# ViTAE-Transformer/SAMRS

Hardware: AMD Instinct MI355X
Metric: images/sec (1024^2, vit_h, 32 boxes/img) SAM box->mask (higher is better)
Workload: dtype f16

## Files before the change

### include/samrs_hip.h

```cpp
#ifndef SAMRS_HIP_H
#define SAMRS_HIP_H

#include <stdint.h>

#ifdef __cplusplus
extern "C" {
#endif

#define SAMRS_ABI_VERSION 5

enum samrs_status {
    SAMRS_OK = 0,
    SAMRS_ERR_NOT_SET = -1,
    SAMRS_ERR_BAD_SHAPE = -2,
    SAMRS_ERR_BAD_ARG = -3,
    SAMRS_ERR_HIP = -4,
    SAMRS_ERR_BAD_WEIGHTS = -5,
    SAMRS_ERR_CAPACITY = -6,
    SAMRS_ERR_PRECISION = -7,
    SAMRS_ERR_RANGE = -8
};

enum samrs_precision {
    SAMRS_PREC_BF16 = 0,
// ... 39 lines not shown
int samrs_predict(samrs_engine_t* e, int slot, int n_prompts,
                  const float* boxes, const float* point_coords, const int32_t* point_labels,
                  int n_points, const float* mask_input, int multimask, int return_logits,
                  int in_h, int in_w, int orig_h, int orig_w,
                  void* masks_out, float* iou_out, float* lowres_out, void* stream);

int samrs_predict_multi(samrs_engine_t* e, int n_images, const int* slots, const int* prompt_offsets,
                        const float* boxes, const float* point_coords, const int32_t* point_labels, int n_points,
                        const float* mask_input, int multimask, int return_logits,
                        const int* in_hw, const int* orig_hw, void* const* masks_out, float* iou_out, float* lowres_out,
                        void* stream);

int samrs_paint(samrs_engine_t* e, const uint8_t* masks, const int32_t* labels, int n,
                int orig_h, int orig_w, uint8_t* seg_mask, int64_t* areas_out,
                int64_t* class_pixels, int64_t* class_instances, int n_classes, void* stream);

int samrs_select_best(samrs_engine_t* e, const uint8_t* masks, const float* iou, int n, int n_sel, int h, int w,
                      uint8_t* best_out, float* quality_out, int64_t* areas_out, void* stream);

int samrs_gt_match(samrs_engine_t* e, const uint8_t* masks, int n, int h, int w, const uint8_t* label_rgb,
                   const uint8_t* colors, int64_t* inter_out, int64_t* gt_area_out, uint8_t* gt_masks_out, void* stream);

int samrs_rle_encode(samrs_engine_t* e, const uint8_t* masks, int n, int h, int w, uint8_t* out, int64_t out_capacity,
                     int64_t* cursor, int64_t* table, void* stream);

int samrs_scene_claim(samrs_engine_t* e, const uint8_t* masks, const int32_t* ranks, const int32_t* labels, int n, int h, int w,
                      int x0, int y0, int H, int W, int32_t* order, int64_t* areas_out,
                      int64_t* class_pixels, int64_t* class_instances, int n_classes, void* stream);
int samrs_scene_resolve(samrs_engine_t* e, const int32_t* order, const int32_t* labels_by_rank, int n_ranks, int H, int W,
                        uint8_t* seg, void* stream);
// ... 48 lines not shown
```

### samrs_amd/csrc/decoder_kernels.hip

```cpp
#include "common.h"
#include "kernels.h"
#include "postprocess_value.h"

namespace {

constexpr float TWO_PI = 6.283185307179586f;

__device__ __forceinline__ float pe_channel(const float* __restrict__ gauss, float cx01, float cy01, int ch, int half) {
    const int f = ch < half ? ch : ch - half;
    const float vx = 2.0f * cx01 - 1.0f, vy = 2.0f * cy01 - 1.0f;
    const float a = TWO_PI * (vx * gauss[f] + vy * gauss[half + f]);
    return ch < half ? sinf(a) : cosf(a);
}

__global__ void prompt_tokens_kernel(PromptParams p, float* __restrict__ tokens, float* __restrict__ tokens2, int T, int C) {
    const int j = blockIdx.x, b = blockIdx.y, ch = threadIdx.x;
    const int half = C / 2;
    const bool has_pts = p.point_coords != nullptr;
    const bool has_box = p.boxes != nullptr;
    const int npt = has_pts ? p.n_points + (has_box ? 0 : 1) : 0;
    float v;
    if (j == 0) {
        v = p.iou_token[ch];
    } else if (j < 5) {
// ... 168 lines not shown
#pragma unroll
            for (int c = 0; c < DH; ++c) acc[c] = acc[c] * corr + pj * vr[c];
            m = mn;
        }
        const float inv = 1.0f / l;
        float* orow = o + ((size_t)b * T + i) * C + h * DH;
#pragma unroll
        for (int c = 0; c < DH; ++c) orow[c] = acc[c] * inv;
    }
}

constexpr int T2I_TG = 8;
constexpr int T2I_REC = 10;
constexpr float T2I_NEG = -1.0e30f;

template <int PREC>
__global__ __launch_bounds__(256, 2) void t2i_partial_kernel(const float* __restrict__ qp, const uint16_t* __restrict__ kp,
                                                          const uint16_t* __restrict__ vp, int ld, long bstride,
                                                          const int* __restrict__ slot_of, float* __restrict__ part, int T, int tokens, int Ci, int kpw) {
    __shared__ float sm[4][T2I_TG][16][T2I_REC];
    const int split = blockIdx.x, b = blockIdx.y, t0 = blockIdx.z * T2I_TG;
    const int lane = threadIdx.x & 63, wave = threadIdx.x >> 6;
    const int ch = lane & 15, kq = lane >> 4;
    float q[T2I_TG][8], acc[T2I_TG][8], m[T2I_TG], l[T2I_TG];
#pragma unroll
    for (int t = 0; t < T2I_TG; ++t) {
        m[t] = T2I_NEG;
        l[t] = 0.f;
        const bool tv = t0 + t < T;
        const float* qr = qp + ((size_t)b * T + (tv ? t0 + t : 0)) * Ci + ch * 8;
#pragma unroll
        for (int c = 0; c < 8; ++c) {
            q[t][c] = tv ? qr[c] * (0.25f * 1.44269504088896340736f) : 0.f;
            acc[t][c] = 0.f;
        }
    }
    const int kbeg = (split * 4 + wave) * kpw;
    const int kend = kbeg + kpw < tokens ? kbeg + kpw : tokens;
    const int kbat = slot_of ? slot_of[b] : b;
    const uint16_t* kb = kp + (size_t)kbat * bstride * ld + ch * 8;
    const uint16_t* vb = vp + (size_t)kbat * bstride * ld + ch * 8;
// ... 13 lines not shown
        T2I_LOAD(kn, vn, k0 + 4 * U)
#pragma unroll
        for (int u = 0; u < U; ++u) {
            const bool valid = k0 + 4 * u + kq < kend;
            const uint32_t kw[4] = {kk[u].x, kk[u].y, kk[u].z, kk[u].w};
            const uint32_t vw[4] = {vv[u].x, vv[u].y, vv[u].z, vv[u].w};
            float kf[8], vf[8];
#pragma unroll
            for (int c = 0; c < 4; ++c) {
                kf[2 * c] = ET<PREC>::to_float((uint16_t)(kw[c] & 0xffffu));
                kf[2 * c + 1] = ET<PREC>::to_float((uint16_t)(kw[c] >> 16));
                vf[2 * c] = ET<PREC>::to_float((uint16_t)(vw[c] & 0xffffu));
                vf[2 * c + 1] = ET<PREC>::to_float((uint16_t)(vw[c] >> 16));
            }
#pragma unroll
            for (int t = 0; t < T2I_TG; ++t) {
                float sc = 0.f;
#pragma unroll
                for (int c = 0; c < 8; ++c) sc += q[t][c] * kf[c];
                sc += __builtin_bit_cast(float, __builtin_amdgcn_update_dpp(0, __builtin_bit_cast(int, sc), 0xB1, 0xF, 0xF, true));
                sc = valid ? sc : T2I_NEG;
                const float mn = fmaxf(m[t], sc);
                const float corr = __builtin_amdgcn_exp2f(m[t] - mn);
                const float pj = valid ? __builtin_amdgcn_exp2f(sc - mn) : 0.f;
                l[t] = l[t] * corr + pj;
#pragma unroll
                for (int c = 0; c < 8; ++c) acc[t][c] = acc[t][c] * corr + pj * vf[c];
                m[t] = mn;
            }
        }
#pragma unroll
        for (int u = 0; u < U; ++u) { kk[u] = kn[u]; vv[u] = vn[u]; }
    }
#undef T2I_LOAD
#pragma unroll
    for (int off = 16; off <= 32; off <<= 1) {
#pragma unroll
        for (int t = 0; t < T2I_TG; ++t) {
            const float mo = __shfl_xor(m[t], off, 64), lo = __shfl_xor(l[t], off, 64);
            const float mn = fmaxf(m[t], mo);
            const float fs = __builtin_amdgcn_exp2f(m[t] - mn), fo = __builtin_amdgcn_exp2f(mo - mn);
            l[t] = l[t] * fs + lo * fo;
#pragma unroll
            for (int c = 0; c < 8; ++c) acc[t][c] = acc[t][c] * fs + __shfl_xor(acc[t][c], off, 64) * fo;
            m[t] = mn;
        }
    }
    if (lane < 16) {
#pragma unroll
        for (int t = 0; t < T2I_TG; ++t) {
            float* r = sm[wave][t][ch];
            r[0] = m[t]; r[1] = l[t];
#pragma unroll
            for (int c = 0; c < 8; ++c) r[2 + c] = acc[t][c];
        }
    }
    __syncthreads();
    if (threadIdx.x < T2I_TG * 16) {
        const int t = threadIdx.x >> 4, c16 = threadIdx.x & 15;
        float mm = sm[0][t][c16][0];
#pragma unroll
        for (int w = 1; w < 4; ++w) mm = fmaxf(mm, sm[w][t][c16][0]);
        float ll = 0.f, a[8] = {0.f, 0.f, 0.f, 0.f, 0.f, 0.f, 0.f, 0.f};
#pragma unroll
        for (int w = 0; w < 4; ++w) {
            const float f = __builtin_amdgcn_exp2f(sm[w][t][c16][0] - mm);
            ll += sm[w][t][c16][1] * f;
#pragma unroll
            for (int c = 0; c < 8; ++c) a[c] += sm[w][t][c16][2 + c] * f;
        }
        float* r = part + ((((size_t)b * gridDim.z + blockIdx.z) * gridDim.x + split) * (T2I_TG * 16) + threadIdx.x) * T2I_REC;
        r[0] = mm; r[1] = ll;
#pragma unroll
        for (int c = 0; c < 8; ++c) r[2 + c] = a[c];
    }
}

__global__ __launch_bounds__(T2I_TG * 16) void t2i_merge_kernel(const float* __restrict__ part, float* __restrict__ o,
                                                                int splits, int T, int Ci) {
    const int b = blockIdx.x, tg = blockIdx.y;
    const int t = tg * T2I_TG + (threadIdx.x >> 4), ch = threadIdx.x & 15;
    if (t >= T) return;
    const float* base = part + (((size_t)b * gridDim.y + tg) * splits * (T2I_TG * 16) + threadIdx.x) * T2I_REC;
    const size_t sstride = (size_t)(T2I_TG * 16) * T2I_REC;
    float mm = T2I_NEG;
    for (int s = 0; s < splits; ++s) mm = fmaxf(mm, base[s * sstride]);
// ... 629 lines not shown
    }
}

__global__ void class_stats_kernel(const unsigned long long* __restrict__ areas, const int32_t* __restrict__ labels, int n,
                                   unsigned long long* __restrict__ cpix, unsigned long long* __restrict__ cins, int n_classes) {
    if (threadIdx.x != 0 || blockIdx.x != 0) return;
    for (int j = 0; j < n; ++j) {
        const int l = labels[j];
        if (areas[j] > 0 && l >= 0 && l < n_classes) {
            if (cpix) cpix[l] += areas[j];
            if (cins) cins[l] += 1ull;
        }
    }
}

__global__ void resample_pass_kernel(const uint8_t* __restrict__ in, uint8_t* __restrict__ out, const int32_t* __restrict__ bounds,
                                     const int32_t* __restrict__ coef, int ksize, int in_len, int out_len, int other,
                                     int horizontal) {
    const long t = (long)blockIdx.x * blockDim.x + threadIdx.x;
    const long total = (long)out_len * other * 3;
    if (t >= total) return;
    const int c = t % 3;
    long u = t / 3;
    int o, q;
    if (horizontal) { o = u % out_len; q = u / out_len; } else { q = u % other; o = u / other; }
    const int k0 = bounds[2 * o], kn = bounds[2 * o + 1];
    const int32_t* k = coef + (size_t)o * ksize;
    int ss = 1 << 21;
    for (int i = 0; i < kn; ++i) {
        const size_t idx = horizontal ? ((size_t)q * in_len + (k0 + i)) * 3 + c : ((size_t)(k0 + i) * other + q) * 3 + c;
// ... 163 lines not shown
    if (C / heads != 32 || T > TOK_MAX) return hipErrorInvalidValue;
    token_self_attn_kernel<32><<<n, 256, 3 * T * C * sizeof(float), s>>>(q, k, v, o, T, C, heads);
    return hipGetLastError();
}
size_t t2i_workspace_floats(int n, int T) {
    return (size_t)n * ((T + T2I_TG - 1) / T2I_TG) * T2I_MAX_SPLITS * (T2I_TG * 16) * T2I_REC;
}
hipError_t launch_t2i_attention(int prec, const float* qp, const void* kp, const void* vp, int ld, long bstride,
                                float* o, float* workspace, int n, int T, int tokens, int Ci, int heads, hipStream_t s,
                                const int* slot_of) {
    if (Ci != 128 || heads != 8 || T > TOK_MAX || !workspace) return hipErrorInvalidValue;
    int splits = (tokens + 255) / 256;
    splits = splits < 1 ? 1 : (splits > T2I_MAX_SPLITS ? T2I_MAX_SPLITS : splits);
    const int kpw = ((tokens + splits * 4 - 1) / (splits * 4) + 15) / 16 * 16;
    const int tgs = (T + T2I_TG - 1) / T2I_TG;
    dim3 g(splits, n, tgs), b(256);
    const uint16_t* k = (const uint16_t*)kp;
    const uint16_t* v = (const uint16_t*)vp;
    if (prec == PREC_BF16) t2i_partial_kernel<PREC_BF16><<<g, b, 0, s>>>(qp, k, v, ld, bstride, slot_of, workspace, T, tokens, Ci, kpw);
    else t2i_partial_kernel<PREC_F16><<<g, b, 0, s>>>(qp, k, v, ld, bstride, slot_of, workspace, T, tokens, Ci, kpw);
    t2i_merge_kernel<<<dim3(n, tgs), T2I_TG * 16, 0, s>>>(workspace, o, splits, T, Ci);
    return hipGetLastError();
}
hipError_t launch_i2t_attention(int prec, const void* qi, int ld, long bstride, const float* kt, const float* vt,
                                void* out, int n, int T, int tokens, int Ci, int heads, hipStream_t s) {
    if (Ci / heads != 16 || 256 % heads) return hipErrorInvalidValue;
    const int per = 256 / heads;
    dim3 g((tokens + per - 1) / per, n), b(256);
    const size_t sh = 2 * (size_t)T * heads * I2T_HS * sizeof(float);
    if (prec == PREC_BF16)
        i2t_attention_kernel<PREC_BF16><<<g, b, sh, s>>>((const uint16_t*)qi, ld, bstride, kt, vt, (uint16_t*)out, T, tokens, Ci);
    else
        i2t_attention_kernel<PREC_F16><<<g, b, sh, s>>>((const uint16_t*)qi, ld, bstride, kt, vt, (uint16_t*)out, T, tokens, Ci);
    return hipGetLastError();
}
// ... 64 lines not shown
    const bool fused = seg && areas && hw % 16 == 0 && (((uintptr_t)masks | (uintptr_t)seg) & 15) == 0;
    if (seg && !fused) paint_kernel<<<(int)((hw + 255) / 256), 256, 0, s>>>(masks, labels, n, hw, seg);
    if (areas) {
        HIP_CHECK_RET(hipMemsetAsync(areas, 0, sizeof(unsigned long long) * n, s));
        if (fused) {
            paint_area_kernel<<<(int)((hw / 16 + 255) / 256), 256, 0, s>>>(masks, labels, n, hw, seg, areas);
        } else {
            dim3 g(64, n);
            area_kernel<<<g, 256, 0, s>>>(masks, hw, areas);
        }
        if (class_pixels || class_instances)
            class_stats_kernel<<<1, 64, 0, s>>>(areas, labels, n, class_pixels, class_instances, n_classes);
    }
    return hipGetLastError();
}

hipError_t launch_select_best(const uint8_t* masks, const float* iou, int n, int nsel, int h, int w, uint8_t* out, float* quality,
                              unsigned long long* areas, hipStream_t s) {
    if (n < 1 || nsel < 1 || h < 1 || w < 1) return hipErrorInvalidValue;
    const long hw = (long)h * w;
    HIP_CHECK_RET(hipMemsetAsync(areas, 0, sizeof(unsigned long long) * n, s));
    int chunks = (int)((hw / 16 + 255) / 256);
    chunks = chunks < 1 ? 1 : (chunks > 64 ? 64 : chunks);
    select_best_kernel<<<dim3(chunks, n), 256, 0, s>>>(masks, iou, nsel, hw, out, quality, areas);
    return hipGetLastError();
}

hipError_t launch_gt_match(const uint8_t* masks, int n, int h, int w, const uint8_t* label_rgb, const uint8_t* colors,
                           unsigned long long* inter, unsigned long long* gt_area, uint8_t* gt_masks, hipStream_t s) {
    const long hw = (long)h * w;
// ... 18 lines not shown
```

### samrs_amd/csrc/engine_masks.hip

```cpp
#include <cmath>

#include "engine_state.h"

extern "C" {
int samrs_paint(samrs_engine_t* e, const uint8_t* masks, const int32_t* labels, int n, int h, int w, uint8_t* seg,
                int64_t* areas, int64_t* cpix, int64_t* cins, int n_classes, void* stream) {
    if (!e || !masks || !labels || n < 1 || h < 1 || w < 1) return fail(e, SAMRS_ERR_BAD_ARG, "samrs_paint: bad argument");
    if ((cpix || cins) && !areas) return fail(e, SAMRS_ERR_BAD_ARG, "samrs_paint: class statistics need areas_out");
    ON_DEVICE(e);
    CK(e, launch_paint(masks, labels, n, h, w, seg, (unsigned long long*)areas, (unsigned long long*)cpix,
                       (unsigned long long*)cins, n_classes, (hipStream_t)stream));
    return SAMRS_OK;
}

int samrs_select_best(samrs_engine_t* e, const uint8_t* masks, const float* iou, int n, int n_sel, int h, int w, uint8_t* best_out,
                      float* quality_out, int64_t* areas_out, void* stream) {
    if (!e || !masks || !iou || !best_out || !quality_out || !areas_out || n < 1 || n_sel < 1 || h < 1 || w < 1)
        return fail(e, SAMRS_ERR_BAD_ARG, "samrs_select_best: bad argument");
    ON_DEVICE(e);
    CK(e, launch_select_best(masks, iou, n, n_sel, h, w, best_out, quality_out, (unsigned long long*)areas_out, (hipStream_t)stream));
    return SAMRS_OK;
}
int samrs_gt_match(samrs_engine_t* e, const uint8_t* masks, int n, int h, int w, const uint8_t* label_rgb, const uint8_t* colors,
                   int64_t* inter_out, int64_t* gt_area_out, uint8_t* gt_masks_out, void* stream) {
    if (!e || !masks || !label_rgb || !colors || !inter_out || !gt_area_out || n < 1 || h < 1 || w < 1)
        return fail(e, SAMRS_ERR_BAD_ARG, "samrs_gt_match: bad argument");
// ... 198 lines not shown
```

### samrs_amd/csrc/kernels.h

```cpp
#pragma once
#include <hip/hip_runtime.h>
#include <stdint.h>

struct GemmOpts {
    int ld = 0;
    int gelu_form = 1;
};
hipError_t launch_gemm_et(int prec, const void* A, const void* B, void* C, const float* bias,
                          const float* add2d, int add2d_period, int M, int N, int K, bool out_f32,
                          bool gelu, bool accumulate, hipStream_t s, GemmOpts opts = {});
void gemm_debug_choice(int prec, int M, int N, int K, bool out_f32, bool gelu, bool accumulate, bool has_add2d, int ld, int variant,
                       int32_t* out8);
hipError_t launch_gemm_et_gln(int prec, const void* A, const void* B, void* C, const float* bias, const float* gamma_beta,
                              int M, int N, int K, hipStream_t s, const void* A_lo = nullptr, const void* B_lo = nullptr);
hipError_t launch_gemm_et_stats(int prec, const void* A, const void* B, float* C, const float* bias, void* Xh, float* stats,
                                int M, int N, int K, hipStream_t s);
hipError_t launch_gemm_et_fold(int prec, const void* Xh, const void* Wf, void* C, const float* bias_f, const float* cvec,
                               const float* rowstat, int M, int N, int K, bool gelu, hipStream_t s);
bool gemm_split3_ok(int M, int N, int K, bool out_f32 = false);
hipError_t launch_gemm_et_split3(int prec, const void* A, const void* A_lo, const void* B, const void* B_lo, void* C, const float* bias,
                                 int M, int N, int K, bool out_f32, bool accumulate, hipStream_t s, int split_from_n = 0,
                                 const float* add2d = nullptr, int add2d_period = 0);
void set_gemm_variant(int v);
bool gemm_has_experiments();
// ... 87 lines not shown
                                float* out, float* workspace, int n, int T, int tokens, int Ci, int heads, hipStream_t s,
                                const int* slot_of = nullptr);
hipError_t launch_i2t_attention(int prec, const void* qi, int ld, long batch_stride_rows, const float* kt,
                                const float* vt, void* out, int n, int T, int tokens, int Ci, int heads, hipStream_t s);
hipError_t launch_group_ln_gelu(int prec, const float* in, const float* gamma, const float* beta, float eps,
                                void* out, long rows, int groups, int gsize, hipStream_t s);
hipError_t launch_upscale2_masks(int prec, const void* u1, const void* w, const void* w_lo, const float* bias, const float* hyper,
                                 float* low, int n, int grid, int n_mask_tokens, int sel0, int n_sel, hipStream_t s);
hipError_t launch_mask_product(int prec, const void* up2, const float* hyper, float* low, int n, int grid,
                               int n_mask_tokens, int sel0, int n_sel, hipStream_t s);
hipError_t launch_postprocess(const float* low, int n_masks, int in_h, int in_w, int orig_h, int orig_w,
                              int img_size, int return_logits, void* out, hipStream_t s);
hipError_t launch_paint(const uint8_t* masks, const int32_t* labels, int n, int h, int w, uint8_t* seg,
                        unsigned long long* areas, unsigned long long* class_pixels,
                        unsigned long long* class_instances, int n_classes, hipStream_t s);
hipError_t launch_select_best(const uint8_t* masks, const float* iou, int n, int nsel, int h, int w, uint8_t* out, float* quality,
                              unsigned long long* areas, hipStream_t s);
hipError_t launch_gt_match(const uint8_t* masks, int n, int h, int w, const uint8_t* label_rgb, const uint8_t* colors,
                           unsigned long long* inter, unsigned long long* gt_area, uint8_t* gt_masks, hipStream_t s);
hipError_t launch_resample_pass(const uint8_t* in, uint8_t* out, const int32_t* bounds, const int32_t* coef, int ksize,
                                int in_len, int out_len, int other, int horizontal, hipStream_t s);
hipError_t launch_rbox_prompt(const int32_t* pts, int n, int nv, int h, int w, int th, int tw, int img_size, int out_size,
                              float* out, hipStream_t s,
                              int fill_rule = 0 );
hipError_t launch_i2t_fused(int prec, const void* qi, int ld, long q_bstride, const float* kt, const float* vt, const void* w,
                            const void* w_lo , const float* bias, const float* resid,
                            long r_bstride, const float* gamma, const float* beta, float eps, float* outF, void* outE,
                            void* outE_lo , int n, int T, int tokens, int Ci, int C, hipStream_t s,
                            const int* slot_of = nullptr);

// ... 61 lines not shown
```

### samrs_amd/driver.py

```python
from __future__ import annotations

import contextlib
import os

import queue
import threading
from dataclasses import dataclass, field
from typing import Callable, Iterable, Iterator, List, NamedTuple, Optional, Sequence, Tuple

import numpy as np
import torch


def shard(items: Sequence, rank: int, world: int) -> List:
    return list(sorted(items))[rank::world]


def box_chunks(n: int, batch_size: int) -> List[Tuple[int, int]]:
    out, start = [], 0
    end = min(n, start + batch_size)
    for _ in range(n // batch_size + 1):
        if start < end:
            out.append((start, end))
        start = end
# ... 405 lines not shown
    if need > hi:
        return False, None, f"a chain of {need} prompts exceeds what the engine accepts ({hi})"
    return True, need, f"decode_prompts raised from {capacity} to {need}"


class TilePipeline:

    BOX_WIDTH = 4

    def __init__(self, sam, n_classes: int, batch: int = 8, box_batch: int = 20, keep_masks: bool = False,
                 out_depth: int = 3, max_boxes: int = 512, device_inputs: bool = False, rle: bool = False,
                 rle_buffer_mb: int = 256, precision="auto", _multimask: bool = False, png_lut: Optional[np.ndarray] = None,
                 png_buffer_mb: Optional[int] = None, batch_decode="auto", min_region_area: int = 0,
                 region_mode: str = "both", mask_boxes: bool = False, quality: bool = False, min_stability: float = 0.0,
                 min_pred_iou: float = 0.0, min_inside_box: float = 0.0, polygons: bool = False, polygon_buffer_mb: int = 64,
                 polygon_max_edges: int = 65536):
        from .transforms import ResizeLongestSide
        lut, poly_vertices = validate_output_options(min_region_area, region_mode, polygons, polygon_buffer_mb, polygon_max_edges, png_lut)
        self.min_region_area, self.region_mode = int(min_region_area), region_mode
        self.thresholds = (float(min_stability), float(min_pred_iou), float(min_inside_box))
        if any(t != t or t < 0 for t in self.thresholds):
            raise ValueError("min_stability, min_pred_iou and min_inside_box must be >= 0 (0 = off)")
        self.filter = any(t > 0 for t in self.thresholds)
        self.quality = bool(quality) or self.filter
        eng = sam.engine
        if eng is None:
            raise RuntimeError("move the model to the GPU first: sam.to('cuda')")
        self.split_mode = self._choose_split(sam, precision, multimask=_multimask)
        self.allow_reduced = _multimask and isinstance(precision, int) and not isinstance(precision, bool)
        self.eng = eng
        if self.split_mode is not None:
            with self._mode():
                pass
        if out_depth < 2:
            raise ValueError("out_depth must be >= 2: batch k-1's results are still on loan to the sink when batch k decodes")
        if eng.max_images < 2 * batch:
            raise ValueError(f"TilePipeline(batch={batch}) needs an engine with max_images >= {2 * batch} "
                             f"(two embedding slot sets); got {eng.max_images}")
        self.sam, self.eng, self.dev = sam, eng, eng.device
        self.batch, self.box_batch, self.keep_masks, self.max_boxes = batch, box_batch, keep_masks, max_boxes
        self.rle = rle
        self.batch_decode, self.batch_decode_reason = self._resolve_batch_decode(batch_decode)
        self.batch_decode_on = self.batch_decode
        self.png = png_lut is not None
        self.side = sam.cfg.img_size
        self.transform = ResizeLongestSide(sam.image_encoder.img_size)
        self.class_pixels = torch.zeros(n_classes, dtype=torch.int64, device=self.dev)
        self.class_instances = torch.zeros(n_classes, dtype=torch.int64, device=self.dev)
        dev, side = self.dev, self.side
        self.s_h2d, self.s_enc, self.s_dec = (torch.cuda.Stream(dev) for _ in range(3))
        self.device_inputs = device_inputs
        self.pin_in = None
        if not device_inputs:
            self.pin_in = [torch.empty(batch, side, side, 3, dtype=torch.uint8).pin_memory() for _ in range(2)]
        self.mask_boxes, self.polygons = bool(mask_boxes), bool(polygons)
        self.dev_in = [torch.empty(batch, side, side, 3, dtype=torch.uint8, device=dev) for _ in range(2)]
        bw = self.BOX_WIDTH
        self.pin_box = [torch.empty(batch * max_boxes, bw, dtype=torch.float32).pin_memory() for _ in range(2)]
# ... 154 lines not shown
    def _decode_multi(self, b: int, tiles, offs):
        per = [self._tile_prompts(b, t, hw, off, nb) for (t, hw), (off, nb) in zip(tiles, offs)]
        args = [None if per[0][j] is None else torch.cat([p[j] for p in per]) for j in range(4)]
        masks, iou, low = self.eng.predict_multi([b * self.batch + i for i in range(len(tiles))], [nb for _, nb in offs], *args,
                                               self.multimask, False, [(int(t.shape[0]), int(t.shape[1])) for t, _ in tiles],
                                               [tuple(hw) for _, hw in tiles])
        return list(zip(masks, iou, low))

    def _chunk_masks(self, b: int, i: int, tile, hw, off: int, s: int, e: int, pre):
        if pre is not None:
            return pre[0][s:e], pre[1][s:e], pre[2][s:e]
        in_size = (int(tile.shape[0]), int(tile.shape[1]))
        return self.eng.predict(b * self.batch + i, *self._tile_prompts(b, tile, hw, off + s, e - s), self.multimask, False, in_size,
                                tuple(hw))

    def _decode_tile(self, b: int, i: int, tile, hw, off: int, nb: int, out: _OutBuf, pre=None) -> None:
        eng, (H, W) = self.eng, hw
        in_size = (int(tile.shape[0]), int(tile.shape[1]))
        native = (H, W) == (self.side, self.side)
        seg = self.seg_dev[b][i] if native else torch.full((H, W), 255, dtype=torch.uint8, device=self.dev)
        kept = []
        for s, e in box_chunks(nb, self.box_batch):
            masks, iou, low = self._chunk_masks(b, i, tile, hw, off, s, e, pre)
            if self.quality:
                self._score(b, i, off, s, e, masks[:, 0], iou, low, in_size, (H, W))
            if self.min_region_area:
                eng.clean_masks(masks[:, 0], self.min_region_area, self.region_mode, areas_out=False,
                                changed_out=self.chg_dev[b][i, s:e])
            if self.mask_boxes:
                eng.mask_boxes(masks[:, 0], (0, 0), self.hbox_dev[b][i, s:e], self.rbox_dev[b][i, s:e], self.rec_dev[b][i, s:e])
            if self.polygons:
                eng.mask_polygons(masks[:, 0], (0, 0), self.polygon_max_edges, self.poly_vert_dev[b], self.poly_ring_dev[b],
                                  self.poly_out.cur[b], self.poly_out.tab[b][off + s:off + e])
            eng.paint(masks[:, 0], self.dev_lab[b][off + s:off + e], seg, self.class_pixels, self.class_instances,
                      areas_out=self.area_dev[b][i, s:e])
            if self.rle:
                eng.rle_encode(masks[:, 0], self.rle_dev[b], self.rle_out.cur[b], self.rle_out.tab[b][off + s:off + e])
            if self.keep_masks:
                kept.append(masks[:, 0].view(torch.uint8))
        if self.png and not native:
            eng.png_encode(seg, self.png_lut, self.png_dev[b], self.png_out.cur[b], self.png_out.tab[b][i:i + 1])
        if native:
            out.seg[i].copy_(seg, non_blocking=True)
        else:
            out.odd[i] = seg.cpu()
        out.masks[i] = torch.cat(kept).cpu() if (self.keep_masks and kept) else None

    STABILITY_OFFSET = 1.0

    def _score(self, b: int, i: int, off: int, s: int, e: int, masks, iou, low, in_size, hw) -> None:
        eng = self.eng
        counts = eng.score_masks(low[:, 0], in_size, hw, self.STABILITY_OFFSET, boxes=self.dev_box[b][off + s:off + e],
                                 counts_out=self.cnt_dev[b][i, s:e])
        self.qual_dev[b][i, s:e].copy_(iou[:, 0])
        if self.filter:
            eng.filter_masks(masks, counts, self.qual_dev[b][i, s:e], *self.thresholds, keep_out=self.keep_dev[b][i, s:e])

    def _input_frame_boxes(self, boxes: torch.Tensor, hw, in_size) -> torch.Tensor:
        if tuple(hw) == tuple(in_size):
            return boxes
        return self.transform.apply_boxes_torch(boxes, hw)

    def _decode(self, b: int, items, tiles, offs, out: _OutBuf):
        with torch.cuda.stream(self.s_dec):
            self.s_dec.wait_event(self.ev_enc[b])
            self.seg_dev[b].fill_(255)
            for st in self.streams:
                st.reset(b)
            with self._mode():
                pre = self._decode_multi(b, tiles, offs) if self.batch_decode and sum(nb for _, nb in offs) else None
                for i, ((t, hw), (off, nb)) in enumerate(zip(tiles, offs)):
                    self._decode_tile(b, i, t, hw, off, nb, out, None if pre is None else pre[i])
            if self.png:
                self._encode_png(b, tiles)
            for t in self.tables:
                out.tables[t.field].copy_(getattr(self, t.dev)[b], non_blocking=True)
            for st in self.streams:
                st.copy_table(b, out)
            self.ev_dec[b].record(self.s_dec)
            out.done.record(self.s_dec)

    def _encode_png(self, b: int, tiles) -> None:
        native = [i for i, (_, hw) in enumerate(tiles) if tuple(hw) == (self.side, self.side)]
        runs: List[List[int]] = []
        for i in native:
            if runs and runs[-1][-1] == i - 1:
                runs[-1].append(i)
# ... 199 lines not shown
```

### samrs_amd/engine.py

```python
from __future__ import annotations

import contextlib
import ctypes as C
import os
from typing import Dict, List, Optional, Sequence, Tuple

import numpy as np
import torch

from .synth import SamConfig

_HERE = os.path.dirname(os.path.abspath(__file__))
LIB_PATH = os.path.join(_HERE, "csrc", "libsamrs_hip.so")

PREC_BF16, PREC_F16 = 0, 1
PRECISIONS = {"bf16": PREC_BF16, "f16": PREC_F16, "fp16": PREC_F16}

ABI_VERSION = 5
REGION_MODES = {"holes": 1, "islands": 2, "both": 3}
SPLIT_PATCH, SPLIT_NECK, SPLIT_OI, SPLIT_UP, SPLIT_DEFAULT = 1, 2, 4, 8, 15
SPLIT_ATTN, SPLIT_MLP, SPLIT_ATTN_V, SPLIT_LIN2, SPLIT_ALL = 16, 32, 64, 128, 255

OK, ERR_NOT_SET, ERR_BAD_SHAPE, ERR_BAD_ARG, ERR_HIP, ERR_BAD_WEIGHTS, ERR_CAPACITY, ERR_PRECISION, ERR_RANGE = 0, -1, -2, -3, -4, -5, -6, -7, -8

# ... 31 lines not shown
    lib.samrs_create.argtypes = [C.POINTER(samrs_config), ip, C.c_char_p, ip]
    lib.samrs_destroy.argtypes = [vp]
    lib.samrs_destroy.restype = None
    lib.samrs_last_error.argtypes = [vp]
    lib.samrs_last_error.restype = C.c_char_p
    lib.samrs_load_weight.argtypes = [vp, C.c_char_p, vp, C.POINTER(C.c_int64), ip]
    lib.samrs_finalize_weights.argtypes = [vp, vp]
    lib.samrs_set_images.argtypes = [vp, vp, ip, ip, ip, ip, vp]
    lib.samrs_set_images_ragged.argtypes = [vp, C.POINTER(vp), C.POINTER(ip), C.POINTER(ip), ip, ip, vp]
    lib.samrs_get_embedding.argtypes = [vp, ip, vp, vp]
    lib.samrs_set_embedding.argtypes = [vp, ip, vp, vp]
    lib.samrs_reset_image.argtypes = [vp, ip]
    lib.samrs_predict.argtypes = [vp, ip, ip, vp, vp, vp, ip, vp, ip, ip, ip, ip, ip, ip, vp, vp, vp, vp]
    lib.samrs_predict_multi.argtypes = PREDICT_MULTI_ARGTYPES
    lib.samrs_paint.argtypes = [vp, vp, vp, ip, ip, ip, vp, vp, vp, vp, ip, vp]
    lib.samrs_debug_encoder_prefix.argtypes = [vp, vp, ip, ip, ip, ip, vp, vp]
    lib.samrs_debug_encoder_prefix.restype = ip
    lib.samrs_debug_time_dominant_kernel.argtypes = [vp, ip]
    lib.samrs_debug_time_dominant_kernel.restype = ip
    lib.samrs_debug_dominant_kernel_time.argtypes = [vp, C.POINTER(C.c_float), C.POINTER(ip), C.POINTER(ip), C.POINTER(ip), C.POINTER(ip)]
    lib.samrs_debug_dominant_kernel_time.restype = ip
    lib.samrs_resample_pass_u8.argtypes = [vp, vp, vp, vp, ip, ip, ip, ip, ip, vp]
    lib.samrs_resample_pass_u8.restype = ip
    lib.samrs_rbox_mask_prompt.argtypes = [vp, ip, ip, ip, ip, ip, ip, ip, ip, vp, vp]
    lib.samrs_rbox_mask_prompt.restype = ip
    lib.samrs_rbox_mask_prompt_rule.argtypes = [vp, ip, ip, ip, ip, ip, ip, ip, ip, ip, vp, vp]
    lib.samrs_rbox_mask_prompt_rule.restype = ip
    lib.samrs_k_gemm.argtypes = [ip, vp, vp, vp, vp, vp, ip, ip, ip, ip, ip, ip, ip, vp]
    lib.samrs_k_gemm_f32.argtypes = [vp, ip, vp, vp, vp, ip, ip, ip, ip, ip, ip, vp]
    lib.samrs_k_gemm_stats.argtypes = [ip, vp, vp, vp, vp, vp, vp, ip, ip, ip, vp]
# ... 693 lines not shown
              class_pixels: Optional[torch.Tensor] = None, class_instances: Optional[torch.Tensor] = None,
              areas_out: Optional[torch.Tensor] = None) -> torch.Tensor:
        m = masks.view(torch.uint8) if masks.dtype == torch.bool else masks
        m = m.reshape(-1, m.shape[-2], m.shape[-1]).contiguous()
        n, h, w = m.shape
        labels = labels.to(dtype=torch.int32, device=self.device).contiguous()
        if areas_out is not None:
            assert areas_out.dtype == torch.int64 and areas_out.is_contiguous() and areas_out.numel() == n and areas_out.is_cuda
        areas = areas_out if areas_out is not None else torch.empty(n, dtype=torch.int64, device=self.device)
        ncls = 0 if class_pixels is None else class_pixels.numel()
        with torch.cuda.device(self.device):
            self._check(self.lib.samrs_paint(self.handle, m.data_ptr(), labels.data_ptr(), n, h, w, seg.data_ptr(),
                                             areas.data_ptr(), _ptr(class_pixels), _ptr(class_instances), ncls, _stream()))
        return areas

    def _check_scene(self, rc: int) -> None:
        if rc == ERR_BAD_ARG:
            raise EngineError(self.lib.samrs_last_error(self.handle).decode())
        self._check(rc)

    def scene_claim(self, masks: torch.Tensor, ranks: torch.Tensor, window: Sequence[int], order: torch.Tensor,
                    labels: Optional[torch.Tensor] = None, class_pixels: Optional[torch.Tensor] = None,
                    class_instances: Optional[torch.Tensor] = None, areas_out: Optional[torch.Tensor] = None) -> torch.Tensor:
        m = masks.view(torch.uint8) if masks.dtype == torch.bool else masks
        m = (m if m.dim() == 3 else m.reshape(-1, m.shape[-2], m.shape[-1])).contiguous()
        n, h, w = m.shape
        x0, y0, ww, wh = (int(v) for v in window)
        if (ww, wh) != (w, h):
            raise ValueError(f"window {tuple(window)} does not have the masks' size {w} x {h}")
        assert order.dtype == torch.int32 and order.dim() == 2 and order.is_cuda and order.is_contiguous()
# ... 44 lines not shown
```

Measured before the change: 149.6.

## Batch per-image paint into one multi-image kernel and trim t2i tail token groups

Adds a paint_batch API and kernel that paints masks and counts areas for up to 16 images per launch. The driver defers per-tile paint calls and issues one batched launch plus a single seg copy, cutting per-tile launch and Python overhead. Separately, the token-to-image attention partial kernel is templated on the token count so a ragged tail group runs in a smaller kernel instead of padding a full group; an env var can disable this. The cost is more launches for the t2i tail and added API and validation code paths.

```diff
diff --git a/include/samrs_hip.h b/include/samrs_hip.h
--- a/include/samrs_hip.h
+++ b/include/samrs_hip.h
@@ -77,6 +77,10 @@
 int samrs_paint(samrs_engine_t* e, const uint8_t* masks, const int32_t* labels, int n,
                 int orig_h, int orig_w, uint8_t* seg_mask, int64_t* areas_out,
                 int64_t* class_pixels, int64_t* class_instances, int n_classes, void* stream);
+int samrs_paint_batch(samrs_engine_t* e, int n_images, const uint8_t* const* masks, const int32_t* n_masks,
+                      const int32_t* const* labels, uint8_t* const* seg_masks, int64_t* const* areas_out,
+                      int orig_h, int orig_w, int64_t* areas_table, int64_t areas_table_len,
+                      int64_t* class_pixels, int64_t* class_instances, int n_classes, void* stream);
 
 int samrs_select_best(samrs_engine_t* e, const uint8_t* masks, const float* iou, int n, int n_sel, int h, int w,
                       uint8_t* best_out, float* quality_out, int64_t* areas_out, void* stream);
diff --git a/samrs_amd/csrc/decoder_kernels.hip b/samrs_amd/csrc/decoder_kernels.hip
--- a/samrs_amd/csrc/decoder_kernels.hip
+++ b/samrs_amd/csrc/decoder_kernels.hip
@@ -1,3 +1,5 @@
+#include <cstdlib>
+
 #include "common.h"
 #include "kernels.h"
 #include "postprocess_value.h"
@@ -206,17 +208,19 @@
 constexpr int T2I_REC = 10;
 constexpr float T2I_NEG = -1.0e30f;
 
-template <int PREC>
+template <int PREC, int NT>
 __global__ __launch_bounds__(256, 2) void t2i_partial_kernel(const float* __restrict__ qp, const uint16_t* __restrict__ kp,
                                                           const uint16_t* __restrict__ vp, int ld, long bstride,
-                                                          const int* __restrict__ slot_of, float* __restrict__ part, int T, int tokens, int Ci, int kpw) {
-    __shared__ float sm[4][T2I_TG][16][T2I_REC];
-    const int split = blockIdx.x, b = blockIdx.y, t0 = blockIdx.z * T2I_TG;
+                                                          const int* __restrict__ slot_of, float* __restrict__ part, int T, int tokens, int Ci, int kpw,
+                                                          int tg0, int tgs) {
+    static_assert(NT >= 2 && NT <= T2I_TG, "token lanes per pass");
+    __shared__ float sm[4][NT][16][T2I_REC];
+    const int split = blockIdx.x, b = blockIdx.y, tg = tg0 + blockIdx.z, t0 = tg * T2I_TG;
     const int lane = threadIdx.x & 63, wave = threadIdx.x >> 6;
     const int ch = lane & 15, kq = lane >> 4;
-    float q[T2I_TG][8], acc[T2I_TG][8], m[T2I_TG], l[T2I_TG];
-#pragma unroll
-    for (int t = 0; t < T2I_TG; ++t) {
+    float q[NT][8], acc[NT][8], m[NT], l[NT];
+#pragma unroll
+    for (int t = 0; t < NT; ++t) {
         m[t] = T2I_NEG;
         l[t] = 0.f;
         const bool tv = t0 + t < T;
@@ -260,7 +264,7 @@
                 vf[2 * c + 1] = ET<PREC>::to_float((uint16_t)(vw[c] >> 16));
             }
 #pragma unroll
-            for (int t = 0; t < T2I_TG; ++t) {
+            for (int t = 0; t < NT; ++t) {
                 float sc = 0.f;
 #pragma unroll
                 for (int c = 0; c < 8; ++c) sc += q[t][c] * kf[c];
@@ -282,7 +286,7 @@
 #pragma unroll
     for (int off = 16; off <= 32; off <<= 1) {
 #pragma unroll
-        for (int t = 0; t < T2I_TG; ++t) {
+        for (int t = 0; t < NT; ++t) {
             const float mo = __shfl_xor(m[t], off, 64), lo = __shfl_xor(l[t], off, 64);
             const float mn = fmaxf(m[t], mo);
             const float fs = __builtin_amdgcn_exp2f(m[t] - mn), fo = __builtin_amdgcn_exp2f(mo - mn);
@@ -294,7 +298,7 @@
     }
     if (lane < 16) {
 #pragma unroll
-        for (int t = 0; t < T2I_TG; ++t) {
+        for (int t = 0; t < NT; ++t) {
             float* r = sm[wave][t][ch];
             r[0] = m[t]; r[1] = l[t];
 #pragma unroll
@@ -302,7 +306,7 @@
         }
     }
     __syncthreads();
-    if (threadIdx.x < T2I_TG * 16) {
+    if (threadIdx.x < NT * 16) {
         const int t = threadIdx.x >> 4, c16 = threadIdx.x & 15;
         float mm = sm[0][t][c16][0];
 #pragma unroll
@@ -315,7 +319,7 @@
 #pragma unroll
             for (int c = 0; c < 8; ++c) a[c] += sm[w][t][c16][2 + c] * f;
         }
-        float* r = part + ((((size_t)b * gridDim.z + blockIdx.z) * gridDim.x + split) * (T2I_TG * 16) + threadIdx.x) * T2I_REC;
+        float* r = part + ((((size_t)b * tgs + tg) * gridDim.x + split) * (T2I_TG * 16) + threadIdx.x) * T2I_REC;
         r[0] = mm; r[1] = ll;
 #pragma unroll
         for (int c = 0; c < 8; ++c) r[2 + c] = a[c];
@@ -975,6 +979,93 @@
     }
 }
 
+constexpr int PB_UNROLL = 8;
+static_assert(PA_CHUNK % PB_UNROLL == 0 && PB_UNROLL % 2 == 0, "a chunk of LDS counters holds whole groups of masks");
+struct PaintBatchArgs {
+    const uint8_t* masks[PAINT_BATCH_IMAGES];
+    const int32_t* labels[PAINT_BATCH_IMAGES];
+    uint8_t* seg[PAINT_BATCH_IMAGES];
+    unsigned long long* areas[PAINT_BATCH_IMAGES];
+    int n[PAINT_BATCH_IMAGES];
+};
+__global__ __launch_bounds__(256) void paint_area_batch_kernel(const PaintBatchArgs a, long hw) {
+    __shared__ unsigned int cnt_s[PA_CHUNK];
+    const int img = blockIdx.y;
+    const uint8_t* __restrict__ masks = a.masks[img];
+    const int32_t* __restrict__ labels = a.labels[img];
+    unsigned long long* __restrict__ areas = a.areas[img];
+    const int n = a.n[img];
+    const long p0 = ((long)blockIdx.x * 256 + threadIdx.x) * 16;
+    const bool in = p0 < hw;
+    uint32_t done[4] = {0u, 0u, 0u, 0u}, res[4] = {0u, 0u, 0u, 0u};
+    for (int jhi = n; jhi > 0; jhi -= PA_CHUNK) {
+        const int jlo = jhi > PA_CHUNK ? jhi - PA_CHUNK : 0;
+        if (threadIdx.x < PA_CHUNK) cnt_s[threadIdx.x] = 0u;
+        __syncthreads();
+        for (int j0 = jhi; j0 > jlo; j0 -= PB_UNROLL) {
+            uint4 mv[PB_UNROLL];
+#pragma unroll
+            for (int u = 0; u < PB_UNROLL; ++u) {
+                const int j = j0 - 1 - u;
+                mv[u] = make_uint4(0u, 0u, 0u, 0u);
+                if (in && j >= jlo) mv[u] = *reinterpret_cast<const uint4*>(masks + (size_t)j * hw + p0);
+            }
+            uint32_t packed[PB_UNROLL / 2];
+#pragma unroll
+            for (int u = 0; u < PB_UNROLL / 2; ++u) packed[u] = 0u;
+#pragma unroll
+            for (int u = 0; u < PB_UNROLL; ++u) {
+                const int j = j0 - 1 - u;
+                unsigned int cnt = 0;
+                const uint32_t w[4] = {mv[u].x, mv[u].y, mv[u].z, mv[u].w};
+                const uint32_t lab = (uint32_t)(uint8_t)labels[j >= jlo ? j : jlo] * 0x01010101u;
+#pragma unroll
+                for (int k = 0; k < 4; ++k) {
+                    const uint32_t t = nonzero_bytes(w[k]);
+                    cnt += __popc(t);
+                    const uint32_t mm = (t >> 7) * 0xFFu, fresh = mm & ~done[k];
+                    res[k] = (res[k] & ~fresh) | (fresh & lab);
+                    done[k] |= mm;
+                }
+                packed[u >> 1] |= cnt << (16 * (u & 1));
+            }
+#pragma unroll
+            for (int u = 0; u < PB_UNROLL / 2; ++u) {
+#pragma unroll
+                for (int off = 32; off > 0; off >>= 1) packed[u] += __shfl_xor(packed[u], off, 64);
+            }
+            if ((threadIdx.x & 63) == 0) {
+#pragma unroll
+                for (int u = 0; u < PB_UNROLL; ++u) {
+                    const unsigned int c = (packed[u >> 1] >> (16 * (u & 1))) & 0xFFFFu;
+                    if (c) atomicAdd(&cnt_s[j0 - 1 - u - jlo], c);
+                }
+            }
+        }
+        __syncthreads();
+        if (threadIdx.x < jhi - jlo && cnt_s[threadIdx.x]) atomicAdd(&areas[jlo + threadIdx.x], (unsigned long long)cnt_s[threadIdx.x]);
+        __syncthreads();
+    }
+    if (in && (done[0] | done[1] | done[2] | done[3])) {
+        uint4* sp = reinterpret_cast<uint4*>(a.seg[img] + p0);
+        uint4 o = *sp;
+        o.x = (o.x & ~done[0]) | res[0]; o.y = (o.y & ~done[1]) | res[1];
+        o.z = (o.z & ~done[2]) | res[2]; o.w = (o.w & ~done[3]) | res[3];
+        *sp = o;
+    }
+}
+__global__ __launch_bounds__(256) void class_stats_batch_kernel(const PaintBatchArgs a, unsigned long long* __restrict__ cpix,
+                                                                unsigned long long* __restrict__ cins, int n_classes) {
+    const int img = blockIdx.y, j = blockIdx.x * 256 + threadIdx.x;
+    if (j >= a.n[img]) return;
+    const int l = a.labels[img][j];
+    const unsigned long long ar = a.areas[img][j];
+    if (ar > 0 && l >= 0 && l < n_classes) {
+        if (cpix) atomicAdd(&cpix[l], ar);
+        if (cins) atomicAdd(&cins[l], 1ull);
+    }
+}
+
 __global__ void resample_pass_kernel(const uint8_t* __restrict__ in, uint8_t* __restrict__ out, const int32_t* __restrict__ bounds,
                                      const int32_t* __restrict__ coef, int ksize, int in_len, int out_len, int other,
                                      int horizontal) {
@@ -1168,11 +1259,29 @@
     splits = splits < 1 ? 1 : (splits > T2I_MAX_SPLITS ? T2I_MAX_SPLITS : splits);
     const int kpw = ((tokens + splits * 4 - 1) / (splits * 4) + 15) / 16 * 16;
     const int tgs = (T + T2I_TG - 1) / T2I_TG;
-    dim3 g(splits, n, tgs), b(256);
     const uint16_t* k = (const uint16_t*)kp;
     const uint16_t* v = (const uint16_t*)vp;
-    if (prec == PREC_BF16) t2i_partial_kernel<PREC_BF16><<<g, b, 0, s>>>(qp, k, v, ld, bstride, slot_of, workspace, T, tokens, Ci, kpw);
-    else t2i_partial_kernel<PREC_F16><<<g, b, 0, s>>>(qp, k, v, ld, bstride, slot_of, workspace, T, tokens, Ci, kpw);
+    static const int trim = [] { const char* e = getenv("SAMRS_T2I_TRIM"); return (e && atoi(e) == 0) ? 0 : 1; }();
+    const int full = trim ? T / T2I_TG : tgs, tail = trim ? T - full * T2I_TG : 0;
+#define T2I_GO(P, NT_, TG0, NTG)                                                                                                \
+    t2i_partial_kernel<P, NT_><<<dim3(splits, n, NTG), 256, 0, s>>>(qp, k, v, ld, bstride, slot_of, workspace, T, tokens, Ci, kpw, TG0, tgs)
+#define T2I_ALL(P)                                                                                                              \
+    do {                                                                                                                        \
+        if (full) T2I_GO(P, T2I_TG, 0, full);                                                                                   \
+        switch (tail) {                                                                                                         \
+            case 1:           \
+            case 2: T2I_GO(P, 2, full, 1); break;                                                                               \
+            case 3: T2I_GO(P, 3, full, 1); break;                                                                               \
+            case 4: T2I_GO(P, 4, full, 1); break;                                                                               \
+            case 5: T2I_GO(P, 5, full, 1); break;                                                                               \
+            case 6: T2I_GO(P, 6, full, 1); break;                                                                               \
+            case 7: T2I_GO(P, 7, full, 1); break;                                                                               \
+            default: break;                                                                                                     \
+        }                                                                                                                       \
+    } while (0)
+    if (prec == PREC_BF16) T2I_ALL(PREC_BF16); else T2I_ALL(PREC_F16);
+#undef T2I_ALL
+#undef T2I_GO
     t2i_merge_kernel<<<dim3(n, tgs), T2I_TG * 16, 0, s>>>(workspace, o, splits, T, Ci);
     return hipGetLastError();
 }
@@ -1267,6 +1376,39 @@
     }
     return hipGetLastError();
 }
+hipError_t launch_paint_batch(int n_images, const uint8_t* const* masks, const int* n_masks, const int32_t* const* labels,
+                              uint8_t* const* segs, unsigned long long* const* areas, int h, int w,
+                              unsigned long long* areas_table, long areas_table_len, unsigned long long* class_pixels,
+                              unsigned long long* class_instances, int n_classes, hipStream_t s) {
+    const long hw = (long)h * w;
+    const long chunks = (hw / 16 + 255) / 256;
+    if (areas_table && areas_table_len > 0)
+        HIP_CHECK_RET(hipMemsetAsync(areas_table, 0, sizeof(unsigned long long) * (size_t)areas_table_len, s));
+    PaintBatchArgs a = {};
+    int cnt = 0, max_n = 0;
+    auto flush = [&]() -> hipError_t {
+        if (!cnt) return hipSuccess;
+        paint_area_batch_kernel<<<dim3((unsigned)chunks, cnt), 256, 0, s>>>(a, hw);
+        if (class_pixels || class_instances)
+            class_stats_batch_kernel<<<dim3((max_n + 255) / 256, cnt), 256, 0, s>>>(a, class_pixels, class_instances, n_classes);
+        cnt = max_n = 0;
+        return hipGetLastError();
+    };
+    for (int i = 0; i < n_images; ++i) {
+        const int n = n_masks[i];
+        if (n < 1) continue;
+        const bool fast = segs[i] && areas[i] && hw % 16 == 0 && chunks <= 0x7fffffffL && (((uintptr_t)masks[i] | (uintptr_t)segs[i]) & 15) == 0;
+        if (!fast) {
+            HIP_CHECK_RET(launch_paint(masks[i], labels[i], n, h, w, segs[i], areas[i], class_pixels, class_instances, n_classes, s));
+            continue;
+        }
+        if (!areas_table) HIP_CHECK_RET(hipMemsetAsync(areas[i], 0, sizeof(unsigned long long) * n, s));
+        a.masks[cnt] = masks[i]; a.labels[cnt] = labels[i]; a.seg[cnt] = segs[i]; a.areas[cnt] = areas[i]; a.n[cnt] = n;
+        max_n = n > max_n ? n : max_n;
+        if (++cnt == PAINT_BATCH_IMAGES) HIP_CHECK_RET(flush());
+    }
+    return flush();
+}
 
 hipError_t launch_select_best(const uint8_t* masks, const float* iou, int n, int nsel, int h, int w, uint8_t* out, float* quality,
                               unsigned long long* areas, hipStream_t s) {
diff --git a/samrs_amd/csrc/engine_masks.hip b/samrs_amd/csrc/engine_masks.hip
--- a/samrs_amd/csrc/engine_masks.hip
+++ b/samrs_amd/csrc/engine_masks.hip
@@ -10,6 +10,26 @@
     ON_DEVICE(e);
     CK(e, launch_paint(masks, labels, n, h, w, seg, (unsigned long long*)areas, (unsigned long long*)cpix,
                        (unsigned long long*)cins, n_classes, (hipStream_t)stream));
+    return SAMRS_OK;
+}
+int samrs_paint_batch(samrs_engine_t* e, int n_images, const uint8_t* const* masks, const int32_t* n_masks, const int32_t* const* labels,
+                      uint8_t* const* segs, int64_t* const* areas, int h, int w, int64_t* areas_table, int64_t areas_table_len,
+                      int64_t* cpix, int64_t* cins, int n_classes, void* stream) {
+    if (!e || n_images < 0 || h < 1 || w < 1 || (n_images && (!masks || !n_masks || !labels || !segs || !areas)))
+        return fail(e, SAMRS_ERR_BAD_ARG, "samrs_paint_batch: bad argument");
+    if (areas_table && areas_table_len < 0) return fail(e, SAMRS_ERR_BAD_ARG, "samrs_paint_batch: areas_table_len < 0");
+    for (int i = 0; i < n_images; ++i) {
+        if (n_masks[i] < 0) return fail(e, SAMRS_ERR_BAD_ARG, "samrs_paint_batch: n_masks[%d] = %d", i, n_masks[i]);
+        if (n_masks[i] == 0) continue;
+        if (!masks[i] || !labels[i] || !segs[i] || !areas[i])
+            return fail(e, SAMRS_ERR_BAD_ARG, "samrs_paint_batch: image %d: masks, labels, seg_mask and areas_out are all required", i);
+        if (areas_table && (areas[i] < areas_table || areas[i] + n_masks[i] > areas_table + areas_table_len))
+            return fail(e, SAMRS_ERR_BAD_ARG, "samrs_paint_batch: image %d: areas_out lies outside areas_table", i);
+    }
+    ON_DEVICE(e);
+    CK(e, launch_paint_batch(n_images, masks, n_masks, labels, segs, (unsigned long long* const*)areas, h, w,
+                             (unsigned long long*)areas_table, (long)areas_table_len, (unsigned long long*)cpix,
+                             (unsigned long long*)cins, n_classes, (hipStream_t)stream));
     return SAMRS_OK;
 }
 
diff --git a/samrs_amd/csrc/kernels.h b/samrs_amd/csrc/kernels.h
--- a/samrs_amd/csrc/kernels.h
+++ b/samrs_amd/csrc/kernels.h
@@ -125,6 +125,11 @@
 hipError_t launch_paint(const uint8_t* masks, const int32_t* labels, int n, int h, int w, uint8_t* seg,
                         unsigned long long* areas, unsigned long long* class_pixels,
                         unsigned long long* class_instances, int n_classes, hipStream_t s);
+constexpr int PAINT_BATCH_IMAGES = 16;
+hipError_t launch_paint_batch(int n_images, const uint8_t* const* masks, const int* n_masks, const int32_t* const* labels,
+                              uint8_t* const* segs, unsigned long long* const* areas, int h, int w,
+                              unsigned long long* areas_table, long areas_table_len, unsigned long long* class_pixels,
+                              unsigned long long* class_instances, int n_classes, hipStream_t s);
 hipError_t launch_select_best(const uint8_t* masks, const float* iou, int n, int nsel, int h, int w, uint8_t* out, float* quality,
                               unsigned long long* areas, hipStream_t s);
 hipError_t launch_gt_match(const uint8_t* masks, int n, int h, int w, const uint8_t* label_rgb, const uint8_t* colors,
diff --git a/samrs_amd/driver.py b/samrs_amd/driver.py
--- a/samrs_amd/driver.py
+++ b/samrs_amd/driver.py
@@ -443,7 +443,7 @@
                  png_buffer_mb: Optional[int] = None, batch_decode="auto", min_region_area: int = 0,
                  region_mode: str = "both", mask_boxes: bool = False, quality: bool = False, min_stability: float = 0.0,
                  min_pred_iou: float = 0.0, min_inside_box: float = 0.0, polygons: bool = False, polygon_buffer_mb: int = 64,
-                 polygon_max_edges: int = 65536):
+                 polygon_max_edges: int = 65536, batch_paint: bool = True):
         from .transforms import ResizeLongestSide
         lut, poly_vertices = validate_output_options(min_region_area, region_mode, polygons, polygon_buffer_mb, polygon_max_edges, png_lut)
         self.min_region_area, self.region_mode = int(min_region_area), region_mode
@@ -471,6 +471,7 @@
         self.rle = rle
         self.batch_decode, self.batch_decode_reason = self._resolve_batch_decode(batch_decode)
         self.batch_decode_on = self.batch_decode
+        self.batch_paint = bool(batch_paint) and eng.has_paint_batch
         self.png = png_lut is not None
         self.side = sam.cfg.img_size
         self.transform = ResizeLongestSide(sam.image_encoder.img_size)
@@ -655,7 +656,7 @@
         return self.eng.predict(b * self.batch + i, *self._tile_prompts(b, tile, hw, off + s, e - s), self.multimask, False, in_size,
                                 tuple(hw))
 
-    def _decode_tile(self, b: int, i: int, tile, hw, off: int, nb: int, out: _OutBuf, pre=None) -> None:
+    def _decode_tile(self, b: int, i: int, tile, hw, off: int, nb: int, out: _OutBuf, pre=None, paint_later: Optional[list] = None) -> None:
         eng, (H, W) = self.eng, hw
         in_size = (int(tile.shape[0]), int(tile.shape[1]))
         native = (H, W) == (self.side, self.side)
@@ -673,8 +674,11 @@
             if self.polygons:
                 eng.mask_polygons(masks[:, 0], (0, 0), self.polygon_max_edges, self.poly_vert_dev[b], self.poly_ring_dev[b],
                                   self.poly_out.cur[b], self.poly_out.tab[b][off + s:off + e])
-            eng.paint(masks[:, 0], self.dev_lab[b][off + s:off + e], seg, self.class_pixels, self.class_instances,
-                      areas_out=self.area_dev[b][i, s:e])
+            if paint_later is not None:
+                paint_later.append((i, masks[:, 0], self.dev_lab[b][off + s:off + e], self.area_dev[b][i, s:e]))
+            else:
+                eng.paint(masks[:, 0], self.dev_lab[b][off + s:off + e], seg, self.class_pixels, self.class_instances,
+                          areas_out=self.area_dev[b][i, s:e])
             if self.rle:
                 eng.rle_encode(masks[:, 0], self.rle_dev[b], self.rle_out.cur[b], self.rle_out.tab[b][off + s:off + e])
             if self.keep_masks:
@@ -682,7 +686,8 @@
         if self.png and not native:
             eng.png_encode(seg, self.png_lut, self.png_dev[b], self.png_out.cur[b], self.png_out.tab[b][i:i + 1])
         if native:
-            out.seg[i].copy_(seg, non_blocking=True)
+            if paint_later is None:
+                out.seg[i].copy_(seg, non_blocking=True)
         else:
             out.odd[i] = seg.cpu()
         out.masks[i] = torch.cat(kept).cpu() if (self.keep_masks and kept) else None
@@ -710,8 +715,17 @@
                 st.reset(b)
             with self._mode():
                 pre = self._decode_multi(b, tiles, offs) if self.batch_decode and sum(nb for _, nb in offs) else None
+                later = [] if (self.batch_paint and not self.INSTANCE and pre is not None
+                               and all(tuple(hw) == (self.side, self.side) and nb <= self.box_batch for (_, hw), (_, nb) in zip(tiles, offs))) else None
+                kw = {} if later is None else {"paint_later": later}
                 for i, ((t, hw), (off, nb)) in enumerate(zip(tiles, offs)):
-                    self._decode_tile(b, i, t, hw, off, nb, out, None if pre is None else pre[i])
+                    self._decode_tile(b, i, t, hw, off, nb, out, None if pre is None else pre[i], **kw)
+                if later is not None:
+                    if later:
+                        self.eng.paint_batch([m for _, m, _, _ in later], [l for _, _, l, _ in later], [self.seg_dev[b][i] for i, _, _, _ in later],
+                                             self.class_pixels, self.class_instances, areas_out=[a for _, _, _, a in later],
+                                             areas_table=self.area_dev[b])
+                    out.seg[:len(tiles)].copy_(self.seg_dev[b][:len(tiles)], non_blocking=True)
             if self.png:
                 self._encode_png(b, tiles)
             for t in self.tables:
diff --git a/samrs_amd/engine.py b/samrs_amd/engine.py
--- a/samrs_amd/engine.py
+++ b/samrs_amd/engine.py
@@ -69,6 +69,10 @@
     lib.samrs_predict.argtypes = [vp, ip, ip, vp, vp, vp, ip, vp, ip, ip, ip, ip, ip, ip, vp, vp, vp, vp]
     lib.samrs_predict_multi.argtypes = PREDICT_MULTI_ARGTYPES
     lib.samrs_paint.argtypes = [vp, vp, vp, ip, ip, ip, vp, vp, vp, vp, ip, vp]
+    if hasattr(lib, "samrs_paint_batch"):
+        lib.samrs_paint_batch.argtypes = [vp, ip, C.POINTER(vp), C.POINTER(C.c_int32), C.POINTER(vp), C.POINTER(vp), C.POINTER(vp), ip, ip,
+                                          vp, C.c_int64, vp, vp, ip, vp]
+        lib.samrs_paint_batch.restype = ip
     lib.samrs_debug_encoder_prefix.argtypes = [vp, vp, ip, ip, ip, ip, vp, vp]
     lib.samrs_debug_encoder_prefix.restype = ip
     lib.samrs_debug_time_dominant_kernel.argtypes = [vp, ip]
@@ -792,6 +796,47 @@
                                              areas.data_ptr(), _ptr(class_pixels), _ptr(class_instances), ncls, _stream()))
         return areas
 
+    @property
+    def has_paint_batch(self) -> bool:
+        return hasattr(self.lib, "samrs_paint_batch")
+
+    def paint_batch(self, masks: Sequence[torch.Tensor], labels: Sequence[torch.Tensor], segs: Sequence[torch.Tensor],
+                    class_pixels: Optional[torch.Tensor] = None, class_instances: Optional[torch.Tensor] = None,
+                    areas_out: Optional[Sequence[torch.Tensor]] = None, areas_table: Optional[torch.Tensor] = None) -> List[torch.Tensor]:
+        n_img = len(masks)
+        assert len(labels) == n_img and len(segs) == n_img and (areas_out is None or len(areas_out) == n_img)
+        ms, labs, areas, hw = [], [], [], None
+        for i in range(n_img):
+            m = masks[i].view(torch.uint8) if masks[i].dtype == torch.bool else masks[i]
+            m = m.reshape(-1, m.shape[-2], m.shape[-1]).contiguous()
+            assert m.is_cuda and m.dtype == torch.uint8
+            if hw is None:
+                hw = (int(m.shape[1]), int(m.shape[2]))
+            assert tuple(m.shape[1:]) == hw, "paint_batch: the tiles of one call have one size"
+            lab = labels[i].to(dtype=torch.int32, device=self.device).contiguous()
+            assert lab.numel() == m.shape[0]
+            seg = segs[i]
+            assert seg.dtype == torch.uint8 and seg.is_cuda and seg.is_contiguous() and tuple(seg.shape) == hw
+            if areas_out is not None:
+                a = areas_out[i]
+                assert a.dtype == torch.int64 and a.is_contiguous() and a.numel() == m.shape[0] and a.is_cuda
+            else:
+                a = torch.empty(m.shape[0], dtype=torch.int64, device=self.device)
+            ms.append(m), labs.append(lab), areas.append(a)
+        if n_img == 0:
+            return areas
+        if areas_table is not None:
+            assert areas_table.dtype == torch.int64 and areas_table.is_contiguous() and areas_table.is_cuda and areas_out is not None
+        pa = C.c_void_p * n_img
+        ncls = 0 if class_pixels is None else class_pixels.numel()
+        with torch.cuda.device(self.device):
+            self._check(self.lib.samrs_paint_batch(
+                self.handle, n_img, pa(*[m.data_ptr() for m in ms]), (C.c_int32 * n_img)(*[int(m.shape[0]) for m in ms]),
+                pa(*[t.data_ptr() for t in labs]), pa(*[t.data_ptr() for t in segs]), pa(*[t.data_ptr() for t in areas]), hw[0], hw[1],
+                _ptr(areas_table), 0 if areas_table is None else areas_table.numel(), _ptr(class_pixels), _ptr(class_instances), ncls,
+                _stream()))
+        return areas
+
     def _check_scene(self, rc: int) -> None:
         if rc == ERR_BAD_ARG:
             raise EngineError(self.lib.samrs_last_error(self.handle).decode())
```

Result: no change. 149.6 (median of 2 runs) (+0.0%).
